# hypre-space/hypredrive

Hardware: AMD Instinct MI355X
Metric: DOF/s, AMG-PCG solve phase, 3D 7-pt Laplacian (higher is better)
Workload: dtype f64

## Files before the change

hypredrive_amd/_lib.py:

```python
import ctypes as C
import os

import numpy as np

_HERE = os.path.dirname(os.path.abspath(__file__))
_LIBPATH = os.path.join(_HERE, "lib", "libhypredrv_amd.so")
_L = None


class LibraryError(RuntimeError):
    pass


class AmgParams(C.Structure):
    _fields_ = [("coarsen_type", C.c_int), ("interp_type", C.c_int), ("pmax", C.c_int),
                ("trunc_factor", C.c_double), ("strong_th", C.c_double),
                ("max_row_sum", C.c_double), ("max_coarse_size", C.c_int),
                ("min_coarse_size", C.c_int), ("max_levels", C.c_int),
                ("relax_down", C.c_int), ("relax_up", C.c_int), ("relax_coarse", C.c_int),
                ("sweeps_down", C.c_int), ("sweeps_up", C.c_int), ("sweeps_coarse", C.c_int),
                ("relax_weight", C.c_double), ("outer_weight", C.c_double),
                ("seed", C.c_uint64), ("num_functions", C.c_int),
                ("cheby_order", C.c_int), ("cheby_eig_est", C.c_int), ("cheby_variant", C.c_int), ("cheby_scale", C.c_int),
                ("cheby_fraction", C.c_double),
# ... 43 lines not shown
                ("frelax_type", C.c_int), ("frelax_sweeps", C.c_int), ("grelax_type", C.c_int), ("grelax_sweeps", C.c_int),
                ("frelax_amg", C.POINTER(AmgParams)),
                ("ilu_tri_solve", C.c_int), ("ilu_lower_it", C.c_int), ("ilu_upper_it", C.c_int),
                ("coarse_ilu_max_iter", C.c_int), ("coarse_ilu_tri_solve", C.c_int), ("coarse_ilu_lower_it", C.c_int), ("coarse_ilu_upper_it", C.c_int),
                ("frelax_krylov", C.c_int), ("frelax_krylov_precond", C.c_int), ("frelax_kp", KrylovParams),
                ("coarse_krylov", C.c_int), ("coarse_krylov_precond", C.c_int), ("coarse_kp", KrylovParams),
                ("mgr_cycle", C.c_int), ("mgr_frelax_pos", C.c_int), ("mgr_gsmooth_pos", C.c_int), ("grelax_blocks", C.c_int),
                ("coarse_type", C.c_int), ("nonglk_max_elmts", C.c_int), ("coarse_th", C.c_double)]


SYMBOLS = [
    "hda_last_error", "hda_device_count", "hda_device_name", "hda_device_pci_bus_id", "hda_device_sync",
    "hda_amg_default_params", "hda_krylov_default_params", "hda_csr_create", "hda_csr_destroy",
    "hda_csr_dims", "hda_csr_download", "hda_lap7_create", "hda_spmv", "hda_relax", "hda_dot",
    "hda_l1_norms", "hda_strength", "hda_pmis", "hda_interp_extpi", "hda_interp_direct", "hda_rap", "hda_transpose",
    "hda_spgemm", "hda_amg_create", "hda_amg_destroy", "hda_amg_num_levels",
    "hda_last_precond_calls", "hda_amg_create_dof", "hda_format_bytes", "hda_probe_spmv", "hda_probe_read", "hda_amg_level_matrix", "hda_amg_fold_sweep", "hda_amg_level_cf", "hda_amg_complexities", "hda_amg_vcycle_bytes",
    "hda_amg_vcycle", "hda_pcg", "hda_gmres", "hda_time_kernel", "hda_solve_device",
    "hda_pcg_iteration_bytes", "hda_memory_stats", "hda_memory_cached", "hda_memory_driver_stats", "hda_memory_trim", "hda_comm_selftest", "hda_check_row_total", "hda_ilu_create", "hda_ilu_create_blocks", "hda_ilu_blocks", "hda_ilu_factors", "hda_fgmres", "hda_bicgstab", "hda_mgr_create", "hda_mgr_matrix", "hda_mgr_blk_inverses",
    "hda_probe_add", "hda_probe_read_id", "hda_borrow_hypredrv", "hda_comm_stats", "hda_comm_name", "hda_comm_size", "hda_halo_plan_host",
    "hda_amd_partitioned_levels", "hda_amd_hierarchy_levels",
    "hda_second_strength", "hda_coarsen_second_pass", "hda_interp_multipass", "hda_truncate_rows", "hda_interp_agg_two_stage",
    "hda_interp_mm_extpi", "hda_interp_extended", "hda_interp_mm_ext", "hda_interp_one_point", "hda_interp_standard", "hda_set_overlap", "hda_marker", "hda_relax_blocks", "hda_l1_norms_blocks", "hda_hmis_blocks", "hda_amg_blocks", "hda_amg_level_blocks",
    "hda_csr_form", "hda_spmv_mode", "hda_air_restriction",
    "hda_cljp", "hda_rs_blocks", "hda_falgout_blocks", "hda_measure_rnd",
    "hda_schwarz_create", "hda_schwarz_domains", "hda_schwarz_info", "hda_precond_time",
    "hda_spgemm_last_route", "hda_sort_rows_last_route",
    "hda_ams_default_amg_params", "hda_ams_create", "hda_ams_matrix", "hda_ams_info",
]


TESTRANKS_SYMBOLS = ["hda_thread_ranks_lap7", "hda_thread_world_create", "hda_thread_world_join", "hda_thread_world_leave",
                     "hda_thread_world_destroy", "hda_testranks_selftest"]
_TESTRANKS_PATH = os.path.join(os.path.dirname(_LIBPATH), "libhypredrv_amd_testranks.so")
_T = None


def load_testranks():
    global _T
    if _T is None:
        load()
        if not os.path.exists(_TESTRANKS_PATH):
            raise LibraryError(f"{_TESTRANKS_PATH} not built: run `python -c 'import __graft_entry__ as g; g.build()'`")
        _T = C.CDLL(_TESTRANKS_PATH)
    return _T


# ... 82 lines not shown
    L.hda_set_overlap.argtypes = [C.c_int]
    L.hda_set_overlap.restype = None
    L.hda_amg_num_levels.argtypes = [vp]
    L.hda_amg_level_matrix.argtypes = [vp, C.c_int, C.c_int, P(vp)]
    L.hda_amg_level_cf.argtypes = [vp, C.c_int, ip]
    L.hda_amg_fold_sweep.argtypes = [vp, C.c_int, dp, dp, dp, dp, dp]
    L.hda_amg_complexities.argtypes = [vp, dp, dp]
    L.hda_amg_vcycle_bytes.argtypes = [vp]
    L.hda_amg_vcycle_bytes.restype = C.c_double
    L.hda_amg_vcycle.argtypes = [vp, dp, dp]
    for f in (L.hda_pcg, L.hda_gmres, L.hda_fgmres, L.hda_bicgstab):
        f.argtypes = [vp, vp, P(KrylovParams), dp, dp, dp, ip, ip, dp]
    L.hda_time_kernel.argtypes = [C.c_int, vp, vp, C.c_int, dp, dp]
    L.hda_solve_device.argtypes = [vp, vp, P(KrylovParams), C.c_int, dp, C.c_int, dp, ip, dp, dp, dp, dp]
    L.hda_pcg_iteration_bytes.argtypes = [vp]
    L.hda_pcg_iteration_bytes.restype = C.c_double
    L.hda_memory_stats.argtypes = [dp, dp]
    L.hda_memory_cached.restype = C.c_double
    L.hda_memory_driver_stats.argtypes = [C.POINTER(C.c_double), C.c_int]
    L.hda_check_row_total.argtypes = [C.c_longlong, C.c_int]
    L.hda_format_bytes.argtypes = [vp, vp, dp, dp, dp, ip]
    L.hda_probe_spmv.argtypes = [vp, C.c_int]
    L.hda_csr_form.argtypes = [vp, C.c_int, ip]
    L.hda_air_restriction.argtypes = [vp, ip, C.c_int, C.c_double, C.c_double, P(vp), P(C.c_int64)]
    L.hda_spmv_mode.argtypes = [vp, C.c_int, C.c_int, C.c_double, C.c_double, dp, dp, dp, dp, dp, dp, dp, dp, dp, ip]
    L.hda_probe_read.argtypes = [dp, ip]
    L.hda_probe_add.argtypes = [vp, C.c_int, ip]
    L.hda_probe_read_id.argtypes = [C.c_int, dp, ip]
    L.hda_borrow_hypredrv.argtypes = [vp, P(vp), P(vp)]
    L.hda_comm_stats.argtypes = [dp, C.c_int]
    L.hda_comm_name.restype = C.c_char_p
    _L = L
    return L


def _check(rc):
    if rc != 0:
        raise LibraryError(f"libhypredrv_amd error {rc}: {load().hda_last_error().decode()}")


def _dp(a):
    return a.ctypes.data_as(C.POINTER(C.c_double))


def _ip(a):
    return a.ctypes.data_as(C.POINTER(C.c_int))
# ... 657 lines not shown
            "windowed": d.value in (3, 5), "value_coded": d.value in (4, 5)}


FORMS = {-1: "none", 0: "lane_group", 1: "stream", 2: "window", 3: "window_runs", 4: "coded", 5: "rowclass"}
SPMV_MODES = {"plain": 0, "plain_dot": 1, "resid": 2, "jacobi": 3, "jacobi_dot": 4, "scaled_copy": 5}


def air_restriction(A, cf, distance=2, strong_th=0.25, filter_th=0.0):
    cfa = np.ascontiguousarray(np.concatenate([np.asarray(cf, dtype=np.int32), np.zeros(1, np.int32)]), dtype=np.int32)
    st = np.zeros(5, dtype=np.int64)
    out = C.c_void_p()
    _check(load().hda_air_restriction(A.h, _ip(cfa), int(distance), float(strong_th), float(filter_th), C.byref(out),
                                      st.ctypes.data_as(C.POINTER(C.c_int64))))
    return Csr(out), dict(fallback=int(st[0]), max_m=int(st[1]), small=int(st[2]), mid=int(st[3]), large=int(st[4]))


def csr_form(A, nown=-1):
    info = np.zeros(8, dtype=np.int32)
    _check(load().hda_csr_form(A.h, nown, _ip(info)))
    return dict(kernel=FORMS[int(info[0])], lpr=int(info[1]), value_coded=bool(info[2]), escapes=int(info[3]),
                rc_esc_rows=int(info[4]), maxrow=int(info[5]), blocks=int(info[6]), vc_packed=int(info[7]))


def spmv_mode(A, mode, x, nown=-1, alpha=1.0, beta=0.0, yin=None, in_place=False, b=None, dinv=None, w=None, dinv2=None, y2=None):
    n = A.nrows
    f64 = lambda v: None if v is None else np.ascontiguousarray(v, dtype=np.float64)
    x, yin, b, dinv, w, dinv2 = f64(x), f64(yin), f64(b), f64(dinv), f64(w), f64(dinv2)
    y = yin.copy() if in_place else np.zeros(n)
    y2 = (np.zeros(n) if y2 is None else f64(y2).copy()) if dinv2 is not None else None
    p = lambda v: None if v is None else _dp(v)
    dot, taken = C.c_double(), C.c_int()
    _check(load().hda_spmv_mode(A.h, SPMV_MODES[mode], nown, alpha, beta, p(x), _dp(y) if in_place else p(yin), p(b), p(dinv), p(w),
                                p(dinv2), _dp(y), p(y2), C.byref(dot), C.byref(taken)))
    return dict(y=y, y2=y2, dot=dot.value, epilogue_taken=bool(taken.value))


def probe_spmv(A, mode):
    _check(load().hda_probe_spmv(A.h if A is not None else None, mode))


def probe_read():
    ms, n = C.c_double(), C.c_int()
    _check(load().hda_probe_read(C.byref(ms), C.byref(n)))
    return ms.value, n.value


# ... 130 lines not shown
```

hypredrive_amd/csrc/hda_capi.hip:

```cpp
#include "../../include/hypredrv_amd.h"

#include "hda_krylov.h"
#include "hda_comm.h"
#include "hda_hypre.h"

#include <chrono>
#include <cmath>
#include <cstring>

using namespace hda;

struct hda_csr_s {
   DCsr           m;
   DArray<double> rhs;
   bool           borrowed = false;
   const DCsr    *ref      = nullptr;
   const double  *rhs_ref  = nullptr;
   const HaloPlan *halo    = nullptr;
   const DCsr    &get() const { return ref ? *ref : m; }
};
struct hda_amg_s {
   Amg                                    *amg = nullptr;
   std::unique_ptr<Amg>                    owned_amg;
   std::unique_ptr<Ilu>                    ilu;
// ... 1383 lines not shown
   dx.upload(x, nc);
   dy.upload(y, nr);
   const bool in_place = yin == y;
   if (mode == HDA_SPMV_PLAIN && yin && !in_place) dyin.upload(yin, nr);
   if (b) db.upload(b, nr);
   if (dinv) ddinv.upload(dinv, nr);
   if (w) dw.upload(w, nr);
   if (mode == HDA_SPMV_SCALED_COPY)
   {
      ddinv2.upload(dinv2, nr);
      dy2.upload(y2, nr);
   }
   const double *pyin = (mode != HDA_SPMV_PLAIN || !yin) ? nullptr : in_place ? dy.data() : dyin.data();
   double        d    = 0.0;
   bool          taken = false;
   spmv_test_mode(m, mode, nown, alpha, beta, dx.data(), pyin, db.data(), ddinv.data(), dw.data(), ddinv2.data(), dy.data(), dy2.data(), &d, &taken);
   dy.download(y, nr);
   if (mode == HDA_SPMV_SCALED_COPY) dy2.download(y2, nr);
   if (dot) *dot = d;
   if (epilogue_taken) *epilogue_taken = taken;
   HDA_CATCH
}

extern "C" int hda_borrow_hypredrv(void *hypredrv, hda_csr_t *A, hda_amg_t *amg)
{
   HDA_TRY
   const DCsr     *m    = nullptr;
   const HaloPlan *halo = nullptr;
   const double   *rhs  = nullptr;
   Amg            *g    = nullptr;
   HDA_REQUIRE(hypredrv_peek(hypredrv, &m, &halo, &rhs, &g) && m, "hda_borrow_hypredrv: the object has no matrix yet");
   if (A)
   {
      auto v      = std::make_unique<hda_csr_s>();
      v->borrowed = true;
      v->ref      = m;
      v->rhs_ref  = rhs;
      v->halo     = halo;
      *A          = v.release();
   }
   if (amg)
   {
      HDA_REQUIRE(g, "hda_borrow_hypredrv: the preconditioner is not a set-up BoomerAMG hierarchy");
      auto h = std::make_unique<hda_amg_s>();
      h->amg = g;
      *amg   = h.release();
// ... 132 lines not shown
```

hypredrive_amd/csrc/hda_kernels.h:

```cpp
#pragma once

#include "hda_common.h"

namespace hda {

struct HaloPlan;


void spmv(const DCsr &A, double alpha, const double *x, double beta, const double *y_in,
          double *y_out, const HaloPlan *halo = nullptr);
bool spmv_with_scaled_copy(const DCsr &A, const double *x, double *y, const double *dinv2, double *y2, const HaloPlan *halo = nullptr);
void spmv_dot(const DCsr &A, const double *x, double *y, const double *w, int slot, const HaloPlan *halo = nullptr);
void residual(const DCsr &A, const double *x, const double *b, double *out, const HaloPlan *halo = nullptr);

void jacobi(const DCsr &A, const double *dinv, const double *b, const double *x_in,
            double *x_out, int dot_slot, const HaloPlan *halo = nullptr, const double *cdinv = nullptr);
bool class_divisors(const DCsr &A, const double *dinv, DArray<double> &table);
const unsigned char *row_classes(const DCsr &A);
void jacobi_folded(const DCsr &A, const DCsr &Pt, const double *dinv, const double *t, const double *e, const double *u, double *out);
bool spmv_foldable(const DCsr &Pt);
void jacobi_zero_guess(int n, const double *dinv, const double *b, double *x);

enum Scalar : int {
   S_GAMMA0 = 0, S_RR0 = 1, S_GAMMA1 = 2, S_RR1 = 3, S_SP = 4, S_BB = 5, S_TMP = 6, S_TMP2 = 7,
   S_GMRES = 8
};
void dot(int n, const double *x, const double *y, int slot);
void finalize(int slot, int scalar_idx);
void finalize_n(int first_slot, int nslots, int first_scalar);
void cg_update(int n, int gamma_idx, const double *p, const double *s, double *x, double *r, int rr_slot, int sp_slot = -1,
               const double *dinv0 = nullptr, double *z0 = nullptr, const unsigned char *rclass = nullptr, const double *cdinv = nullptr);
void cg_direction(int n, int gamma_old_idx, int gamma_new_idx, const double *z, double *p, int first_slot = -1, double *x = nullptr);
void cg_flush_x(int n, int gamma_idx, const double *p, double *x);
void cg_single_step(int n, int t_new, int t_old, int alpha_idx, bool first, const double *u, const double *w, double *p, double *s, double *x,
                    double *r, int rr_slot);
// ... 51 lines not shown
```

hypredrive_amd/csrc/hda_kernels.hip:

```cpp
#include "hda_kernels.h"
#include "hda_sort.h"

#include "hda_dist.h"
#include "hda_mpi_join.h"
#include <unistd.h>

#include <algorithm>
#include <cmath>
#include <cstring>
#include <limits>
#include <map>
#include <mutex>
#include <type_traits>
#include <unordered_map>
#include <rocprim/device/device_segmented_radix_sort.hpp>

namespace hda {


Context::Context()
{
   HDA_HIP(hipGetDevice(&device));
   HDA_HIP(hipStreamCreateWithFlags(&stream, hipStreamNonBlocking));
   {
// ... 987 lines not shown
            o0 = (beta == 0.0) ? alpha * sum[h] : alpha * sum[h] + beta * e0[h];
            if (DOT) acc += o0 * e1[h];
         }
         else if (MODE == MODE_RESID) o0 = e0[h] - sum[h];
         else
         {
            o0 = e2[h] + e1[h] * (e0[h] - sum[h]);
            if (DOT) acc += e0[h] * o0;
         }
         out[r] = o0;
      }
   }
   if (DOT)
   {
      acc = block_sum(acc);
      if (tid == 0)
      {
         partial[blockIdx.x] = acc;
         if (blockIdx.x + gridDim.x < kRedBlocks) partial[blockIdx.x + gridDim.x] = 0.0;
      }
   }
}

template <int MODE, bool DOT, bool SPLIT, bool CD = false>
__global__ __launch_bounds__(256) void k_spmv_rowclass(int nrows, const unsigned char *__restrict__ rclass,
                                                       const unsigned long long *__restrict__ rc_keys, const double *__restrict__ dval,
                                                       const int *__restrict__ ddelta, const int *__restrict__ rowptr,
                                                       const int *__restrict__ col, const double *__restrict__ val,
                                                       const double *__restrict__ x, double alpha, double beta, const double *yin,
                                                       const double *__restrict__ b, const double *__restrict__ dinv,
                                                       const double *__restrict__ w, double *out, double *__restrict__ partial, int nown,
                                                       const double *__restrict__ cdinv = nullptr)
{
   static_assert(!CD || MODE == MODE_JACOBI, "class divisors belong to the Jacobi sweep");
   __shared__ double sv[128 * 8];
   __shared__ int    sd[128 * 8];
   __shared__ int    sn[128];
   __shared__ double sdv[CD ? 128 : 1];
   const int tid = threadIdx.x;
   if (tid < 128)
   {
      if (CD) sdv[tid] = cdinv[tid];
      const unsigned long long key = tid < kRcSlots ? rc_keys[tid] : kRcNoKey;
      int                      n   = 0;
      for (int u = 0; u < 8; u++)
      {
         const unsigned c = (unsigned)(key >> (8 * u)) & 255u;
         const bool     on = key != kRcNoKey && c < 254u;
         sv[tid * 8 + u]   = on ? dval[c] : 0.0;
         sd[tid * 8 + u]   = on ? ddelta[c] : 0;
         n += on;
      }
      sn[tid] = n;
   }
   __syncthreads();
   const int xcd = blockIdx.x & 7, slot = blockIdx.x >> 3, nslot = gridDim.x >> 3;
   const int per = (((nrows + 7) >> 3) + 255) / 256 * 256;
   double    acc = 0.0;
   int    n_cls = 254;
   double n_e0 = 0.0, n_e1 = 0.0, n_e2 = 0.0;
   auto fetch = [&](int tile) {
      const int r = xcd * per + tile * 256 + tid;
      n_cls = 254;
      n_e0 = n_e1 = n_e2 = 0.0;
      if (tile * 256 < per && r < nrows)
      {
         n_cls = (int)rclass[r];
         if (MODE == MODE_PLAIN) { if (beta != 0.0) n_e0 = yin[r]; if (DOT) n_e1 = w[r]; }
         else if (MODE == MODE_RESID) n_e0 = b[r];
         else
         {
            n_e0 = b[r];
            n_e2 = x[r];
            if (!CD || n_cls >= 128) n_e1 = dinv[r];
         }
      }
   };
   fetch(slot);
   for (int tile = slot; tile * 256 < per; tile += nslot)
   {
      const int    r    = xcd * per + tile * 256 + tid;
      const bool   live = r < nrows;
      const int    cls  = n_cls;
      const double e0 = n_e0, e1 = (CD && cls < 128) ? sdv[cls] : n_e1, e2 = n_e2;
      double       sum = 0.0;
      fetch(tile + nslot);
      if (cls < 128)
      {
         const int     n  = sn[cls];
         const double *cv = sv + cls * 8;
         const int    *cd = sd + cls * 8;
         double        xv[8];
#pragma unroll
         for (int u = 0; u < 8; u++)
         {
            const int j = r + cd[u];
            xv[u]       = (u < n && (!SPLIT || j < nown)) ? x[j] : 0.0;
         }
#pragma unroll
         for (int u = 0; u < 8; u++)
         {
            const double t = sum + cv[u] * xv[u];
            sum            = (u < n) ? t : sum;
         }
      }
      else if (cls == 255)
      {
         for (int k = rowptr[r]; k < rowptr[r + 1]; k++)
         {
            const int j = col[k];
            if (!SPLIT || j < nown) sum += val[k] * x[j];
         }
      }
      if (live)
      {
         double o0;
         if (MODE == MODE_PLAIN)
         {
            o0 = (beta == 0.0) ? alpha * sum : alpha * sum + beta * e0;
            if (DOT) acc += o0 * e1;
         }
         else if (MODE == MODE_RESID) o0 = e0 - sum;
         else
         {
            o0 = e2 + e1 * (e0 - sum);
            if (DOT) acc += e0 * o0;
         }
         out[r] = o0;
      }
   }
   if (DOT)
   {
      acc = block_sum(acc);
      if (tid == 0)
      {
         partial[blockIdx.x] = acc;
         if (blockIdx.x + gridDim.x < kRedBlocks) partial[blockIdx.x + gridDim.x] = 0.0;
      }
   }
}
// ... 859 lines not shown
   ensure_forms(A, false);
   if (A.coded == 1) return A.rowcoded == 1 ? SpmvForm::RowClass : SpmvForm::Coded;
   const bool small = !split && A.nnz <= kSmallNnz && A.nnz > 0;
   if (A.maxrow <= kMaxRowLds && !small)
   {
      ensure_forms(A, true, split);
      if (A.win == 1) return A.win_runs ? SpmvForm::WindowRuns : SpmvForm::Window;
      return SpmvForm::Stream;
   }
   return split ? SpmvForm::None : SpmvForm::LaneGroup;
}

struct SpmvCall {
   SpmvCall(const double *x_, double *out_) : x(const_cast<double *>(x_)), out(out_) {}
   double       *x;
   double       *out;
   double        alpha = 1.0, beta = 0.0;
   const double *yin = nullptr, *b = nullptr, *dinv = nullptr, *w = nullptr;
   double       *partial = nullptr;
   const double *dinv2   = nullptr;
   double       *out2    = nullptr;
   const DCsr   *fold    = nullptr;
   const double *cdinv   = nullptr;
};

template <int MODE, bool DOT>
constexpr bool spmv_variant_ok(bool vc, bool split, bool runs, bool epi, bool fold, int pack)
{
   if (epi && (split || MODE != MODE_PLAIN || DOT)) return false;
   if (fold && (vc || runs || split || epi || MODE != MODE_JACOBI || DOT)) return false;
   if (runs && vc) return false;
   if (pack != 0 && (!vc || split || runs)) return false;
   return true;
}

template <auto... Vs>
struct OneOf {
   std::common_type_t<decltype(Vs)...> v;
};
using Flag = OneOf<false, true>;
template <class F>
static void instantiate(F &&f) { f(); }
template <class F, auto... Vs, class... Rest>
static void instantiate(F &&f, OneOf<Vs...> a, Rest... rest)
{
   const bool listed = ((a.v == Vs && (instantiate([&](auto... c) { f(std::integral_constant<decltype(Vs), Vs>{}, c...); }, rest...), true)) || ...);
// ... 2 lines not shown
[[noreturn]] static void spmv_no_kernel() { throw Error("product launch: no kernel exists for this combination of options"); }

template <int MODE, bool DOT>
static bool launch_spmv_impl(const DCsr &A_in, const SpmvCall &c, int nown = -1)
{
   const bool  split = nown >= 0;
   const bool  fold  = MODE == MODE_JACOBI && !DOT && !split && c.fold;
   const DCsr &A     = fold ? *c.fold : A_in;
   if (A.nrows == 0 && !DOT) return fold;
   const SpmvForm form = spmv_form(A, split);
   HDA_REQUIRE(form != SpmvForm::None, "split product on an operator that has no split form");
   HDA_REQUIRE(!fold || fold_form(form, A), "folded sweep armed on an operator whose storage form has no folded kernel");
   const bool stencil = form == SpmvForm::RowClass || form == SpmvForm::Coded;
   const bool runs    = form == SpmvForm::WindowRuns;
   const bool vc      = A.coded == 2 && (form == SpmvForm::Stream || form == SpmvForm::Window);
   const int pack = (vc && form == SpmvForm::Window && A.vc_pack == 1) ? (A.vc_maxesc <= kEscSlotsSmall ? kEscSlotsSmall : kEscCap) : 0;
   HDA_REQUIRE(!(split && pack), "split product on a value-coded operator with packed escapes");
   const bool     epi   = MODE == MODE_PLAIN && !DOT && !split && c.out2 && !stencil;
   const double  *dinv2 = epi ? c.dinv2 : nullptr;
   double        *out2  = epi ? c.out2 : nullptr;
   const auto    *code  = vc ? A.code.data() : nullptr;
   const double  *dict  = vc ? A.dict_val.data() : nullptr;
   const int      gmax  = split ? kOverlapGrid : kRedBlocks;
   if (stencil)
   {
      const int per  = (((A.nrows + 7) >> 3) + 255) / 256 * 256;
      const int grid = DOT ? gmax : std::min(gmax, 8 * (per / 256));
      const bool cd = MODE == MODE_JACOBI && form == SpmvForm::RowClass && c.cdinv;
      instantiate(
         [&](auto SPLIT, auto CD) {
            if constexpr (CD && MODE != MODE_JACOBI) spmv_no_kernel();
            else if (form == SpmvForm::RowClass)
               k_spmv_rowclass<MODE, DOT, SPLIT, CD><<<grid, 256, 0, STREAM>>>(A.nrows, A.rclass.data(), A.rc_keys.data(), A.dict_val.data(),
                                                                               A.dict_delta.data(), A.rowptr.data(), A.col.data(), A.val.data(), c.x,
                                                                               c.alpha, c.beta, c.yin, c.b, c.dinv, c.w, c.out, c.partial, nown,
                                                                               CD ? c.cdinv : nullptr);
            else
               k_spmv_coded_row<MODE, DOT, SPLIT><<<grid, 256, 0, STREAM>>>(A.nrows, A.rowptr.data(), A.code.data(), A.dict_val.data(),
                                                                            A.dict_delta.data(), A.col.data(), A.val.data(), c.x, c.alpha, c.beta,
                                                                            c.yin, c.b, c.dinv, c.w, c.out, c.partial, SPLIT ? nown : 0);
         },
         Flag{split}, Flag{cd});
   }
   else if (form == SpmvForm::Window || form == SpmvForm::WindowRuns)
   {
      const int     plen = kWChunk + A.maxrow;
      const size_t  wlds = sizeof(double) * (size_t)(plen + A.win_maxu);
      const int     wg   = DOT ? gmax : std::min(gmax, ((A.nwin + 7) / 8) * 8);
      const double *val  = pack ? A.vc_esc.data() : A.val.data();
      instantiate(
         [&](auto VC, auto SPLIT, auto RUNS, auto EPI, auto FOLD, auto PACK) {
            if constexpr (spmv_variant_ok<MODE, DOT>(VC, SPLIT, RUNS, EPI, FOLD, PACK))
               k_spmv_win<MODE, DOT, VC, SPLIT, RUNS, EPI, FOLD, PACK><<<wg, 256, wlds, STREAM>>>(
                  A.nwin, A.wmeta.data(), A.rowptr.data(), A.lidx.data(), A.ucol.data(), val, c.x, c.alpha, c.beta, c.yin, c.b, c.dinv, c.w, c.out,
                  c.partial, nown, plen, code, dict, kWinPf, dinv2, out2);
            else spmv_no_kernel();
         },
         Flag{vc}, Flag{split}, Flag{runs}, Flag{epi}, Flag{fold}, OneOf<0, kEscSlotsSmall, kEscCap>{pack});
   }
   else if (form == SpmvForm::Stream)
   {
      const int    grid = DOT ? gmax : std::min(gmax, ((A.nchunks + 7) / 8) * 8);
      const size_t lds  = sizeof(double) * (size_t)(kChunk + A.maxrow);
      instantiate(
         [&](auto VC, auto SPLIT, auto FOLD) {
// ... 169 lines not shown
}

void spmv(const DCsr &A, double alpha, const double *x, double beta, const double *y_in, double *y_out, const HaloPlan *halo)
{
   SpmvCall c(x, y_out);
   c.alpha = alpha;
   c.beta  = beta;
   c.yin   = y_in;
   launch_spmv<MODE_PLAIN, false>(A, halo, c);
}
bool spmv_with_scaled_copy(const DCsr &A, const double *x, double *y, const double *dinv2, double *y2, const HaloPlan *halo)
{
   SpmvCall c(x, y);
   c.dinv2 = dinv2;
   c.out2  = y2;
   return launch_spmv<MODE_PLAIN, false>(A, halo, c);
}
void spmv_dot(const DCsr &A, const double *x, double *y, const double *w, int slot, const HaloPlan *halo)
{
   SpmvCall c(x, y);
   c.w       = w;
   c.partial = Context::get().slot(slot);
   launch_spmv<MODE_PLAIN, true>(A, halo, c);
}
void residual(const DCsr &A, const double *x, const double *b, double *out, const HaloPlan *halo)
{
   SpmvCall c(x, out);
   c.b = b;
   launch_spmv<MODE_RESID, false>(A, halo, c);
}
void jacobi(const DCsr &A, const double *dinv, const double *b, const double *x_in, double *x_out, int dot_slot, const HaloPlan *halo,
            const double *cdinv)
{
   SpmvCall c(x_in, x_out);
   c.b     = b;
   c.dinv  = dinv;
   c.cdinv = cdinv;
   if (dot_slot >= 0)
   {
      c.partial = Context::get().slot(dot_slot);
      launch_spmv<MODE_JACOBI, true>(A, halo, c);
   }
   else launch_spmv<MODE_JACOBI, false>(A, halo, c);
}

__global__ __launch_bounds__(256) void k_cdinv_collect(int n, const unsigned char *__restrict__ rclass, const double *__restrict__ dinv,
// ... 213 lines not shown
               Flag{spp != nullptr}, OneOf<0, 1, 2>{zm});
}

template <bool FIN, bool XUP>
__global__ __launch_bounds__(256) void k_cg_dir(int n, double *scalars, int go, int gn, const double *__restrict__ z, double *__restrict__ p,
                                                const double *__restrict__ partials2, double *__restrict__ x)
{
   double g;
   if (FIN)
   {
      g = slot_sum_256(partials2);
      if (blockIdx.x == 0)
      {
         const double rr = slot_sum_256(partials2 + kRedBlocks);
         if (threadIdx.x == 0) { scalars[gn] = g; scalars[gn + 1] = rr; }
      }
   }
   else g = scalars[gn];
   const double beta  = g / scalars[go];
   const double alpha = XUP ? scalars[go] / scalars[S_SP] : 0.0;
   for (long i = (long)blockIdx.x * 256 + threadIdx.x; i < n; i += (long)gridDim.x * 256)
   {
      const double pi = p[i];
      if (XUP) x[i] += alpha * pi;
      p[i] = z[i] + beta * pi;
   }
}
void cg_direction(int n, int gamma_old_idx, int gamma_new_idx, const double *z, double *p, int first_slot, double *x)
{
   Context &c = Context::get();
   if (first_slot >= 0)
   {
      const int g = std::max(ew_grid(n), 1);
      if (x) k_cg_dir<true, true><<<g, 256, 0, STREAM>>>(n, c.scalars, gamma_old_idx, gamma_new_idx, z, p, c.slot(first_slot), x);
      else k_cg_dir<true, false><<<g, 256, 0, STREAM>>>(n, c.scalars, gamma_old_idx, gamma_new_idx, z, p, c.slot(first_slot), nullptr);
   }
   else if (n)
   {
      if (x) k_cg_dir<false, true><<<ew_grid(n), 256, 0, STREAM>>>(n, c.scalars, gamma_old_idx, gamma_new_idx, z, p, nullptr, x);
      else k_cg_dir<false, false><<<ew_grid(n), 256, 0, STREAM>>>(n, c.scalars, gamma_old_idx, gamma_new_idx, z, p, nullptr, nullptr);
   }
}

__global__ __launch_bounds__(256) void k_cg_flush_x(int n, const double *__restrict__ scalars, int gamma_idx, const double *__restrict__ p,
                                                    double *__restrict__ x)
{
   const double alpha = scalars[gamma_idx] / scalars[S_SP];
   for (long i = (long)blockIdx.x * 256 + threadIdx.x; i < n; i += (long)gridDim.x * 256) x[i] += alpha * p[i];
}
void cg_flush_x(int n, int gamma_idx, const double *p, double *x)
{
   if (n) k_cg_flush_x<<<ew_grid(n), 256, 0, STREAM>>>(n, Context::get().scalars, gamma_idx, p, x);
}

__global__ __launch_bounds__(256) void k_cg_single(int n, double *scalars, int t_new, int t_old, int alpha_idx, int first, const double *__restrict__ u,
                                                   const double *__restrict__ w, double *__restrict__ p, double *__restrict__ s,
                                                   double *__restrict__ x, double *__restrict__ r, double *__restrict__ partial)
{
   const double gn = scalars[t_new], delta = scalars[t_new + 2];
   double       beta = 0.0, alpha;
   if (first) alpha = gn / delta;
   else
   {
      beta  = gn / scalars[t_old];
      alpha = gn / (delta - beta * gn / scalars[alpha_idx]);
   }
   double acc = 0.0;
   for (long i = (long)blockIdx.x * 256 + threadIdx.x; i < n; i += (long)gridDim.x * 256)
   {
      const double pi = u[i] + beta * p[i], si = w[i] + beta * s[i];
      p[i]            = pi;
// ... 660 lines not shown
```

hypredrive_amd/csrc/hda_krylov.hip:

```cpp
#include "hda_krylov.h"

#include <cmath>

namespace hda {

#define g_last_precond_calls (RankState<int, 5>::get())
int last_precond_calls() { return g_last_precond_calls; }

namespace {
struct NestedScope {
   static thread_local int depth;
   DArray<double>          save;
   bool                    nested;
   static constexpr size_t kScal = Context::kNumScalars, kPart = (size_t)Context::kNumSlots * kRedBlocks;
   NestedScope() : nested(depth++ > 0)
   {
      if (!nested) return;
      Context &ctx = Context::get();
      save.alloc(kScal + kPart);
      HDA_HIP(hipMemcpyAsync(save.data(), ctx.scalars, kScal * sizeof(double), hipMemcpyDeviceToDevice, ctx.stream));
      HDA_HIP(hipMemcpyAsync(save.data() + kScal, ctx.partials, kPart * sizeof(double), hipMemcpyDeviceToDevice, ctx.stream));
   }
   ~NestedScope()
   {
      depth--;
      if (!nested) return;
      Context &ctx = Context::get();
      (void)hipMemcpyAsync(ctx.scalars, save.data(), kScal * sizeof(double), hipMemcpyDeviceToDevice, ctx.stream);
      (void)hipMemcpyAsync(ctx.partials, save.data() + kScal, kPart * sizeof(double), hipMemcpyDeviceToDevice, ctx.stream);
   }
};
thread_local int NestedScope::depth = 0;
}

double pcg_iteration_bytes(const DCsr &A, bool format)
{
   const double n = A.nrows;
   const char  *dxe = getenv("HDA_DEFER_X");
   const double vec = (format && !(dxe && atoi(dxe) == 0)) ? 24.0 * n + 40.0 * n : 48.0 * n + 24.0 * n;
   return (matrix_stream_bytes(A, format) + rowptr_stream_bytes(A, format) + 8.0 * A.ncols + 8.0 * n) + 8.0 * n + vec;
}

static KrylovResult pcg_single_reduction(const LinOp &op, const PrecondFn &M, const KrylovParams &kp, const double *b, double *x)
{
   Context     &ctx = Context::get();
   const DCsr  &A   = *op.A;
   const int    n   = A.nrows;
   KrylovResult res;
   const size_t vl = std::max<size_t>(op.veclen, 1);
   DArray<double> r(vl), u(vl), w(vl), p(vl), s(vl);
   constexpr int T0 = S_GMRES, T1 = S_GMRES + 3, S_ALPHA = S_GMRES + 6;
   auto precond = [&](const double *rr, double *zz, int slot) {
      res.precond_calls++;
      if (M) M(rr, zz, slot);
      else
      {
         copy(n, rr, zz);
         if (slot >= 0) dot(n, rr, zz, slot);
      }
   };
   dot(n, b, b, 0);
   finalize(0, S_BB);
// ... 99 lines not shown
      res.precond_calls++;
      fs.valid = false;
      if (M) M(rr, zz, slot);
      else
      {
         copy(n, rr, zz);
         if (slot >= 0) dot(n, rr, zz, slot);
      }
      HDA_REQUIRE(!fs.done, "the preconditioner ignored a first sweep it had offered to take from the caller");
      const bool mine = fs.valid && fs.n == n;
      z0_dinv = mine ? fs.dinv : nullptr;
      z0_dest = mine ? fs.dest : nullptr;
      z0_cdinv  = mine ? fs.cdinv : nullptr;
      z0_rclass = mine ? fs.rclass : nullptr;
      z0_self = mine && fs.dest == nullptr;
      fs.valid = false;
   };
   const char *ffe = getenv("HDA_FUSE_FINALIZE");
   const int   fl  = (Comm::world().size == 1) ? (ffe ? atoi(ffe) : 1) : 0;
   const bool  fin = fl >= 1, fin2 = fl >= 2;
   const char *dxe     = getenv("HDA_DEFER_X");
   const bool  defer_x = !(dxe && atoi(dxe) == 0);
   double     *xd      = defer_x ? x : nullptr;

   double bi_prod;
   if (kp.two_norm && known && !std::isnan(known->bb)) bi_prod = known->bb;
   else
   {
      if (kp.two_norm) dot(n, b, b, 0);
      else precond(b, p.data(), 0);
      finalize(0, S_BB);
      bi_prod = read_scalar(S_BB);
   }
   if (bi_prod == 0.0)
   {
      copy(n, b, x);
      ctx.sync();
      res.hist.push_back(0.0);
      return res;
   }
   double eps = kp.rtol * kp.rtol;
   {
      const double a2 = kp.atol * kp.atol / bi_prod;
      if (a2 > eps) eps = a2;
   }
   if (known && known->x_zero) copy(n, b, r.data());
   else
   {
      copy(n, x, p.data());
      residual(A, p.data(), b, r.data(), op.halo);
   }
   precond(r.data(), p.data(), 2);
   dot(n, r.data(), r.data(), 3);
   finalize_n(2, 2, S_GAMMA0);
   read_scalars_async(S_GAMMA0, 5);
   wait_event(ctx.ev);
   double i_prod = kp.two_norm ? ctx.host_scalars[S_RR0] : ctx.host_scalars[S_GAMMA0];
   res.hist.push_back(std::sqrt(std::fabs(i_prod)));
   int it = 0, x_term = -1;
   std::vector<hipEvent_t> evs;
   static const bool fuse_dots = !(getenv("HDA_FUSE_DOTS") && atoi(getenv("HDA_FUSE_DOTS")) == 0);
   while (it + 1 <= kp.max_iter)
   {
      it++;
      const int go = (it & 1) ? S_GAMMA0 : S_GAMMA1, gn = (it & 1) ? S_GAMMA1 : S_GAMMA0, rn = gn + 1;
      if (kp.profile_k1)
      {
         hipEvent_t e0, e1;
         HDA_HIP(hipEventCreate(&e0));
         HDA_HIP(hipEventCreate(&e1));
         HDA_HIP(hipEventRecord(e0, ctx.stream));
         spmv_dot(A, p.data(), s.data(), p.data(), 0, op.halo);
         HDA_HIP(hipEventRecord(e1, ctx.stream));
         evs.push_back(e0);
         evs.push_back(e1);
      }
      else
         spmv_dot(A, p.data(), s.data(), p.data(), 0, op.halo);
      if (!fin) finalize(0, S_SP);
      double *z0 = z0_dinv ? (z0_self ? s.data() : z0_dest) : nullptr;
      cg_update(n, go, p.data(), s.data(), defer_x ? nullptr : x, r.data(), 3, fin ? 0 : -1, z0_dinv, z0, z0_rclass, z0_cdinv);
      x_term = defer_x ? go : -1;
      bool stop = false;
      auto test = [&]() {
         wait_event(ctx.ev);
         const double sp = ctx.host_scalars[S_SP];
         if (sp == 0.0 || !std::isfinite(sp))
         {
            it--;
            stop = true;
            return;
         }
         i_prod = kp.two_norm ? ctx.host_scalars[rn] : ctx.host_scalars[gn];
         res.hist.push_back(std::sqrt(std::fabs(i_prod)));
         if (kp.print_level >= 2)
            printf("%5d    %e    %f    %e\n", it, res.hist.back(),
                   res.hist[res.hist.size() - 2] > 0 ? res.hist.back() / res.hist[res.hist.size() - 2] : 0.0,
                   std::sqrt(i_prod / bi_prod));
         if (i_prod / bi_prod < eps)
         {
            res.converged = true;
            stop          = true;
         }
      };
      bool near = false;
      if (kp.two_norm && res.hist.size() >= 2)
      {
         const double h1 = res.hist.back(), h0 = res.hist[res.hist.size() - 2];
         const double rho2 = (h0 > 0.0) ? (h1 / h0) * (h1 / h0) : 1.0;
         near = h1 * h1 * rho2 < 16.0 * eps * bi_prod;
      }
      if (near)
      {
         finalize(3, rn);
         read_scalars_async(S_GAMMA0, 5);
         test();
         if (stop) break;
         fs.done = z0 != nullptr;
         fs.in   = r.data();
         fs.out  = s.data();
         precond(r.data(), s.data(), 2);
         if (fin2) cg_direction(n, go, gn, s.data(), p.data(), 2, xd);
         else
         {
            finalize(2, gn);
            cg_direction(n, go, gn, s.data(), p.data(), -1, xd);
         }
         x_term = -1;
         continue;
      }
      if (!fuse_dots) finalize(3, rn);
      fs.done = z0 != nullptr;
      fs.in   = r.data();
      fs.out  = s.data();
      precond(r.data(), s.data(), 2);
      if (fin2 && fuse_dots)
      {
         cg_direction(n, go, gn, s.data(), p.data(), 2, xd);
         read_scalars_async(S_GAMMA0, 5);
      }
      else
      {
         if (fuse_dots) finalize_n(2, 2, gn);
         else finalize(2, gn);
         read_scalars_async(S_GAMMA0, 5);
         cg_direction(n, go, gn, s.data(), p.data(), -1, xd);
      }
      x_term = -1;
      test();
      if (stop) break;
   }
   fs = FirstSweepFusion();
   if (x_term >= 0) cg_flush_x(n, x_term, p.data(), x);
   ctx.sync();
   gs_free_check();
   for (size_t e = 0; e + 1 < evs.size(); e += 2)
   {
      float ms = 0.f;
      if (hipEventElapsedTime(&ms, evs[e], evs[e + 1]) == hipSuccess)
      {
         res.k1_ms_sum += ms;
         res.k1_count++;
      }
      (void)hipEventDestroy(evs[e]);
      (void)hipEventDestroy(evs[e + 1]);
   }
   res.iters     = it;
   res.final_rel = std::sqrt(std::fabs(i_prod) / bi_prod);
   if (!scope.nested) g_last_precond_calls = res.precond_calls;
   return res;
}

static KrylovResult gmres_core(bool flexible, const LinOp &op, const PrecondFn &M, const KrylovParams &kp, const double *b, double *x)
{
   NestedScope  scope;
   Context     &ctx = Context::get();
// ... 210 lines not shown
```

include/hypredrv_amd.h:

```cpp
#ifndef HYPREDRV_AMD_H
#define HYPREDRV_AMD_H

#include <stdint.h>

#ifdef __cplusplus
extern "C" {
#endif

#define HDA_OK 0
#define HDA_ERR_NO_DEVICE 1
#define HDA_ERR_RUNTIME 2
#define HDA_ERR_ARG 3

typedef struct hda_csr_s *hda_csr_t;
typedef struct hda_amg_s *hda_amg_t;

typedef struct {
   int      coarsen_type, interp_type, pmax;
   double   trunc_factor, strong_th, max_row_sum;
   int      max_coarse_size, min_coarse_size, max_levels;
   int      relax_down, relax_up, relax_coarse;
   int      sweeps_down, sweeps_up, sweeps_coarse;
   double   relax_weight, outer_weight;
   uint64_t seed;
// ... 126 lines not shown
int hda_amg_complexities(hda_amg_t h, double *grid, double *op);
double hda_amg_vcycle_bytes(hda_amg_t h);
int hda_amg_vcycle(hda_amg_t h, const double *b, double *x);

int hda_pcg(hda_csr_t A, hda_amg_t amg, const hda_krylov_params *kp, const double *b, double *x,
            double *hist, int *iters, int *converged, double *final_rel);
int hda_gmres(hda_csr_t A, hda_amg_t amg, const hda_krylov_params *kp, const double *b, double *x,
              double *hist, int *iters, int *converged, double *final_rel);
int hda_fgmres(hda_csr_t A, hda_amg_t amg, const hda_krylov_params *kp, const double *b, double *x,
              double *hist, int *iters, int *converged, double *final_rel);
int hda_bicgstab(hda_csr_t A, hda_amg_t amg, const hda_krylov_params *kp, const double *b, double *x,
              double *hist, int *iters, int *converged, double *final_rel);

int hda_time_kernel(int kind, hda_csr_t A, hda_amg_t amg, int reps, double *avg_ms, double *bytes);
int hda_last_precond_calls(void);
int hda_solve_device(hda_csr_t A, hda_amg_t amg, const hda_krylov_params *kp, int solver,
                     const double *b_host, int nsolves, double *solve_ms, int *iters,
                     double *final_rel, double *r0_norm, double *true_rel, double *k1_avg_ms);
double hda_pcg_iteration_bytes(hda_csr_t A);
int hda_format_bytes(hda_csr_t A, hda_amg_t amg, double *pcg_iteration, double *vcycle, double *spmv, int *coded);
enum { HDA_FORM_NONE = -1, HDA_FORM_LANE_GROUP = 0, HDA_FORM_STREAM = 1, HDA_FORM_WINDOW = 2, HDA_FORM_WINDOW_RUNS = 3, HDA_FORM_CODED = 4,
       HDA_FORM_ROWCLASS = 5 };
int hda_csr_form(hda_csr_t A, int nown, int *info);
enum { HDA_SPMV_PLAIN = 0, HDA_SPMV_PLAIN_DOT = 1, HDA_SPMV_RESID = 2, HDA_SPMV_JACOBI = 3, HDA_SPMV_JACOBI_DOT = 4, HDA_SPMV_SCALED_COPY = 5 };
int hda_spmv_mode(hda_csr_t A, int mode, int nown, double alpha, double beta, const double *x, const double *yin, const double *b,
                  const double *dinv, const double *w, const double *dinv2, double *y, double *y2, double *dot, int *epilogue_taken);
int hda_probe_spmv(hda_csr_t A, int mode);
int hda_probe_read(double *avg_ms, int *count);
int hda_probe_add(hda_csr_t A, int mode, int *id);
int hda_probe_read_id(int id, double *avg_ms, int *count);
int hda_borrow_hypredrv(void *hypredrv, hda_csr_t *A, hda_amg_t *amg);
int hda_halo_plan_host(int nloc, const long long *part, const long long *ghost_gids, int nghost, int *send_counts,
                       int *recv_counts, int *send_idx, int send_cap, int *send_total);
int hda_comm_stats(double out[5], int reset);
void hda_set_overlap(int mode);
const char *hda_comm_name(void);
int hda_amd_partitioned_levels(void *hypredrv);
int hda_amd_hierarchy_levels(void *hypredrv);
int         hda_comm_size(void);
int hda_comm_selftest(void);
int hda_memory_stats(double *in_use, double *peak);
double hda_memory_cached(void);
int hda_memory_driver_stats(double out[3], int reset);
int hda_memory_trim(void);
int hda_check_row_total(long long nrows, int row_len);

// ... 5 lines not shown
```

Measured before the change: 592.2 million.

## Fuse the CG direction update into the following row-class SpMV-dot kernel

The PCG loop now defers the p = z + beta*p update (and the deferred x update) and performs it inside the next SpMV-with-dot kernel for single-rank row-class operators. The new p is formed in shared memory for in-tile neighbours and recomputed from z and the old p for far neighbours, with p double-buffered. This removes one full vector pass (read z, p, x; write p, x) per iteration and one kernel launch. In exchange the SpMV reads z and p instead of p alone, adds two block barriers per tile, and needs an extra preconditioner-output buffer and p buffer. A test entry point and explicit rounding intrinsics are added so the fused and unfused paths match bitwise.

```diff
diff --git a/hypredrive_amd/_lib.py b/hypredrive_amd/_lib.py
--- a/hypredrive_amd/_lib.py
+++ b/hypredrive_amd/_lib.py
@@ -89,7 +89,7 @@
     "hda_amd_partitioned_levels", "hda_amd_hierarchy_levels",
     "hda_second_strength", "hda_coarsen_second_pass", "hda_interp_multipass", "hda_truncate_rows", "hda_interp_agg_two_stage",
     "hda_interp_mm_extpi", "hda_interp_extended", "hda_interp_mm_ext", "hda_interp_one_point", "hda_interp_standard", "hda_set_overlap", "hda_marker", "hda_relax_blocks", "hda_l1_norms_blocks", "hda_hmis_blocks", "hda_amg_blocks", "hda_amg_level_blocks",
-    "hda_csr_form", "hda_spmv_mode", "hda_air_restriction",
+    "hda_csr_form", "hda_spmv_mode", "hda_air_restriction", "hda_cg_dir_product",
     "hda_cljp", "hda_rs_blocks", "hda_falgout_blocks", "hda_measure_rnd",
     "hda_schwarz_create", "hda_schwarz_domains", "hda_schwarz_info", "hda_precond_time",
     "hda_spgemm_last_route", "hda_sort_rows_last_route",
@@ -218,6 +218,7 @@
     L.hda_format_bytes.argtypes = [vp, vp, dp, dp, dp, ip]
     L.hda_probe_spmv.argtypes = [vp, C.c_int]
     L.hda_csr_form.argtypes = [vp, C.c_int, ip]
+    L.hda_cg_dir_product.argtypes = [vp, C.c_int, dp, dp, dp, C.c_double, C.c_double, C.c_double, dp, dp, dp, ip]
     L.hda_air_restriction.argtypes = [vp, ip, C.c_int, C.c_double, C.c_double, P(vp), P(C.c_int64)]
     L.hda_spmv_mode.argtypes = [vp, C.c_int, C.c_int, C.c_double, C.c_double, dp, dp, dp, dp, dp, dp, dp, dp, dp, ip]
     L.hda_probe_read.argtypes = [dp, ip]
@@ -921,6 +922,16 @@
                 rc_esc_rows=int(info[4]), maxrow=int(info[5]), blocks=int(info[6]), vc_packed=int(info[7]))
 
 
+def cg_dir_product(A, z, p, x, gamma_old, gamma_new, sp, fused):
+    n = A.nrows
+    z, p = np.ascontiguousarray(z, dtype=np.float64), np.ascontiguousarray(p, dtype=np.float64)
+    xo = None if x is None else np.array(x, dtype=np.float64)
+    pn, s, d, can = np.zeros(n), np.zeros(n), C.c_double(), C.c_int()
+    _check(load().hda_cg_dir_product(A.h, int(bool(fused)), _dp(z), _dp(p), None if xo is None else _dp(xo), float(gamma_old), float(gamma_new),
+                                     float(sp), _dp(pn), _dp(s), C.byref(d), C.byref(can)))
+    return dict(p=pn, s=s, x=xo, dot=d.value, fusable=bool(can.value))
+
+
 def spmv_mode(A, mode, x, nown=-1, alpha=1.0, beta=0.0, yin=None, in_place=False, b=None, dinv=None, w=None, dinv2=None, y2=None):
     n = A.nrows
     f64 = lambda v: None if v is None else np.ascontiguousarray(v, dtype=np.float64)
diff --git a/hypredrive_amd/csrc/hda_capi.hip b/hypredrive_amd/csrc/hda_capi.hip
--- a/hypredrive_amd/csrc/hda_capi.hip
+++ b/hypredrive_amd/csrc/hda_capi.hip
@@ -1429,6 +1429,45 @@
    HDA_CATCH
 }
 
+extern "C" int hda_cg_dir_product(hda_csr_t A, int fused, const double *z, const double *p, double *x, double gamma_old, double gamma_new,
+                                  double sp, double *pnew, double *s, double *dot, int *fusable)
+{
+   HDA_TRY
+   HDA_REQUIRE(A && z && p && pnew && s && dot, "hda_cg_dir_product: null argument");
+   const DCsr &m = A->get();
+   HDA_REQUIRE(m.nrows == m.ncols, "hda_cg_dir_product: square operators only");
+   const bool can = spmv_dir_fusable(m, nullptr);
+   if (fusable) *fusable = can ? 1 : 0;
+   HDA_REQUIRE(!fused || can, "hda_cg_dir_product: the product of this operator has no fused direction step");
+   const size_t   n = (size_t)m.nrows;
+   Context       &ctx = Context::get();
+   DArray<double> dz, dp, dp2(n), ds(n), dx;
+   dz.upload(z, n);
+   dp.upload(p, n);
+   if (x) dx.upload(x, n);
+   const double sc[5] = {gamma_old, 0.0, gamma_new, 0.0, sp};
+   static_assert(S_GAMMA0 == 0 && S_GAMMA1 == 2 && S_SP == 4, "scalar block layout");
+   HDA_HIP(hipMemcpyAsync(ctx.scalars, sc, sizeof(sc), hipMemcpyHostToDevice, ctx.stream));
+   ctx.sync();
+   double *res = dp.data();
+   if (fused)
+   {
+      spmv_dot_dir(m, dz.data(), dp.data(), dp2.data(), ds.data(), x ? dx.data() : nullptr, S_GAMMA0, S_GAMMA1, 0);
+      res = dp2.data();
+   }
+   else
+   {
+      cg_direction((int)n, S_GAMMA0, S_GAMMA1, dz.data(), dp.data(), -1, x ? dx.data() : nullptr);
+      spmv_dot(m, dp.data(), ds.data(), dp.data(), 0, nullptr);
+   }
+   finalize(0, S_TMP);
+   *dot = read_scalar(S_TMP);
+   HDA_HIP(hipMemcpy(pnew, res, n * sizeof(double), hipMemcpyDeviceToHost));
+   ds.download(s, n);
+   if (x) dx.download(x, n);
+   HDA_CATCH
+}
+
 extern "C" int hda_borrow_hypredrv(void *hypredrv, hda_csr_t *A, hda_amg_t *amg)
 {
    HDA_TRY
diff --git a/hypredrive_amd/csrc/hda_kernels.h b/hypredrive_amd/csrc/hda_kernels.h
--- a/hypredrive_amd/csrc/hda_kernels.h
+++ b/hypredrive_amd/csrc/hda_kernels.h
@@ -11,6 +11,8 @@
           double *y_out, const HaloPlan *halo = nullptr);
 bool spmv_with_scaled_copy(const DCsr &A, const double *x, double *y, const double *dinv2, double *y2, const HaloPlan *halo = nullptr);
 void spmv_dot(const DCsr &A, const double *x, double *y, const double *w, int slot, const HaloPlan *halo = nullptr);
+bool spmv_dir_fusable(const DCsr &A, const HaloPlan *halo);
+void spmv_dot_dir(const DCsr &A, const double *z, const double *pold, double *pnew, double *y, double *x, int go, int gn, int slot);
 void residual(const DCsr &A, const double *x, const double *b, double *out, const HaloPlan *halo = nullptr);
 
 void jacobi(const DCsr &A, const double *dinv, const double *b, const double *x_in,
diff --git a/hypredrive_amd/csrc/hda_kernels.hip b/hypredrive_amd/csrc/hda_kernels.hip
--- a/hypredrive_amd/csrc/hda_kernels.hip
+++ b/hypredrive_amd/csrc/hda_kernels.hip
@@ -1033,7 +1033,13 @@
    }
 }
 
-template <int MODE, bool DOT, bool SPLIT, bool CD = false>
+struct CgDirFusion {
+   const double *z = nullptr, *pold = nullptr;
+   double       *pnew = nullptr, *x = nullptr;
+   const double *scalars = nullptr;
+   int           go = 0, gn = 0;
+};
+template <int MODE, bool DOT, bool SPLIT, bool CD = false, bool PRE = false>
 __global__ __launch_bounds__(256) void k_spmv_rowclass(int nrows, const unsigned char *__restrict__ rclass,
                                                        const unsigned long long *__restrict__ rc_keys, const double *__restrict__ dval,
                                                        const int *__restrict__ ddelta, const int *__restrict__ rowptr,
@@ -1041,9 +1047,14 @@
                                                        const double *__restrict__ x, double alpha, double beta, const double *yin,
                                                        const double *__restrict__ b, const double *__restrict__ dinv,
                                                        const double *__restrict__ w, double *out, double *__restrict__ partial, int nown,
-                                                       const double *__restrict__ cdinv = nullptr)
+                                                       const double *__restrict__ cdinv = nullptr, CgDirFusion d = CgDirFusion())
 {
    static_assert(!CD || MODE == MODE_JACOBI, "class divisors belong to the Jacobi sweep");
+   static_assert(!PRE || (MODE == MODE_PLAIN && DOT && !SPLIT), "the direction step rides on the whole plain product with its dot");
+   const double *__restrict__ dz = d.z, *__restrict__ dp = d.pold;
+   const double  dbeta  = PRE ? d.scalars[d.gn] / d.scalars[d.go] : 0.0;
+   const double  dalpha = (PRE && d.x) ? d.scalars[d.go] / d.scalars[S_SP] : 0.0;
+   __shared__ double spn[PRE ? 256 : 1];
    __shared__ double sv[128 * 8];
    __shared__ int    sd[128 * 8];
    __shared__ int    sn[128];
@@ -1077,7 +1088,13 @@
       if (tile * 256 < per && r < nrows)
       {
          n_cls = (int)rclass[r];
-         if (MODE == MODE_PLAIN) { if (beta != 0.0) n_e0 = yin[r]; if (DOT) n_e1 = w[r]; }
+         if (PRE)
+         {
+            n_e0 = dp[r];
+            n_e1 = dz[r];
+            if (d.x) n_e2 = d.x[r];
+         }
+         else if (MODE == MODE_PLAIN) { if (beta != 0.0) n_e0 = yin[r]; if (DOT) n_e1 = w[r]; }
          else if (MODE == MODE_RESID) n_e0 = b[r];
          else
          {
@@ -1095,6 +1112,13 @@
       const int    cls  = n_cls;
       const double e0 = n_e0, e1 = (CD && cls < 128) ? sdv[cls] : n_e1, e2 = n_e2;
       double       sum = 0.0;
+      const double pn = PRE ? __dadd_rn(e1, __dmul_rn(dbeta, e0)) : 0.0;
+      if (PRE)
+      {
+         __syncthreads();
+         spn[tid] = pn;
+         __syncthreads();
+      }
       fetch(tile + nslot);
       if (cls < 128)
       {
@@ -1102,11 +1126,32 @@
          const double *cv = sv + cls * 8;
          const int    *cd = sd + cls * 8;
          double        xv[8];
+         if (PRE)
+         {
+            double zv[8];
 #pragma unroll
-         for (int u = 0; u < 8; u++)
+            for (int u = 0; u < 8; u++)
+            {
+               const int  j   = r + cd[u];
+               const bool far = u < n && (unsigned)(cd[u] + tid) >= 256u;
+               zv[u]          = far ? dz[j] : 0.0;
+               xv[u]          = far ? dp[j] : 0.0;
+            }
+#pragma unroll
+            for (int u = 0; u < 8; u++)
+            {
+               const unsigned o = (unsigned)(cd[u] + tid);
+               xv[u]            = (o < 256u) ? spn[o] : __dadd_rn(zv[u], __dmul_rn(dbeta, xv[u]));
+            }
+         }
+         else
          {
-            const int j = r + cd[u];
-            xv[u]       = (u < n && (!SPLIT || j < nown)) ? x[j] : 0.0;
+#pragma unroll
+            for (int u = 0; u < 8; u++)
+            {
+               const int j = r + cd[u];
+               xv[u]       = (u < n && (!SPLIT || j < nown)) ? x[j] : 0.0;
+            }
          }
 #pragma unroll
          for (int u = 0; u < 8; u++)
@@ -1120,13 +1165,21 @@
          for (int k = rowptr[r]; k < rowptr[r + 1]; k++)
          {
             const int j = col[k];
-            if (!SPLIT || j < nown) sum += val[k] * x[j];
+            if (PRE) sum += val[k] * __dadd_rn(dz[j], __dmul_rn(dbeta, dp[j]));
+            else if (!SPLIT || j < nown) sum += val[k] * x[j];
          }
       }
       if (live)
       {
          double o0;
-         if (MODE == MODE_PLAIN)
+         if (PRE)
+         {
+            d.pnew[r] = pn;
+            if (d.x) d.x[r] = __dadd_rn(e2, __dmul_rn(dalpha, e0));
+            o0 = alpha * sum;
+            acc += o0 * pn;
+         }
+         else if (MODE == MODE_PLAIN)
          {
             o0 = (beta == 0.0) ? alpha * sum : alpha * sum + beta * e0;
             if (DOT) acc += o0 * e1;
@@ -2032,6 +2085,7 @@
    double       *out2    = nullptr;
    const DCsr   *fold    = nullptr;
    const double *cdinv   = nullptr;
+   const CgDirFusion *dir = nullptr;
 };
 
 template <int MODE, bool DOT>
@@ -2080,25 +2134,28 @@
    const auto    *code  = vc ? A.code.data() : nullptr;
    const double  *dict  = vc ? A.dict_val.data() : nullptr;
    const int      gmax  = split ? kOverlapGrid : kRedBlocks;
+   HDA_REQUIRE(!c.dir || stencil, "direction step inside a product that has no kernel for it");
    if (stencil)
    {
       const int per  = (((A.nrows + 7) >> 3) + 255) / 256 * 256;
       const int grid = DOT ? gmax : std::min(gmax, 8 * (per / 256));
       const bool cd = MODE == MODE_JACOBI && form == SpmvForm::RowClass && c.cdinv;
+      const bool pre = c.dir != nullptr;
+      HDA_REQUIRE(!pre || (form == SpmvForm::RowClass && c.beta == 0.0), "direction step inside a product that has no kernel for it");
       instantiate(
-         [&](auto SPLIT, auto CD) {
-            if constexpr (CD && MODE != MODE_JACOBI) spmv_no_kernel();
+         [&](auto SPLIT, auto CD, auto PRE) {
+            if constexpr ((CD && MODE != MODE_JACOBI) || (PRE && !(MODE == MODE_PLAIN && DOT && !SPLIT))) spmv_no_kernel();
             else if (form == SpmvForm::RowClass)
-               k_spmv_rowclass<MODE, DOT, SPLIT, CD><<<grid, 256, 0, STREAM>>>(A.nrows, A.rclass.data(), A.rc_keys.data(), A.dict_val.data(),
-                                                                               A.dict_delta.data(), A.rowptr.data(), A.col.data(), A.val.data(), c.x,
-                                                                               c.alpha, c.beta, c.yin, c.b, c.dinv, c.w, c.out, c.partial, nown,
-                                                                               CD ? c.cdinv : nullptr);
+               k_spmv_rowclass<MODE, DOT, SPLIT, CD, PRE><<<grid, 256, 0, STREAM>>>(A.nrows, A.rclass.data(), A.rc_keys.data(), A.dict_val.data(),
+                                                                                    A.dict_delta.data(), A.rowptr.data(), A.col.data(), A.val.data(),
+                                                                                    c.x, c.alpha, c.beta, c.yin, c.b, c.dinv, c.w, c.out, c.partial,
+                                                                                    nown, CD ? c.cdinv : nullptr, PRE ? *c.dir : CgDirFusion());
             else
                k_spmv_coded_row<MODE, DOT, SPLIT><<<grid, 256, 0, STREAM>>>(A.nrows, A.rowptr.data(), A.code.data(), A.dict_val.data(),
                                                                             A.dict_delta.data(), A.col.data(), A.val.data(), c.x, c.alpha, c.beta,
                                                                             c.yin, c.b, c.dinv, c.w, c.out, c.partial, SPLIT ? nown : 0);
          },
-         Flag{split}, Flag{cd});
+         Flag{split}, Flag{cd}, Flag{pre});
    }
    else if (form == SpmvForm::Window || form == SpmvForm::WindowRuns)
    {
@@ -2314,6 +2371,26 @@
    c.w       = w;
    c.partial = Context::get().slot(slot);
    launch_spmv<MODE_PLAIN, true>(A, halo, c);
+}
+bool spmv_dir_fusable(const DCsr &A, const HaloPlan *halo)
+{
+   return Comm::world().size == 1 && !halo && A.nrows > 0 && spmv_form(A, false) == SpmvForm::RowClass;
+}
+void spmv_dot_dir(const DCsr &A, const double *z, const double *pold, double *pnew, double *y, double *x, int go, int gn, int slot)
+{
+   HDA_REQUIRE(pnew != pold && pnew != z && y != z && y != pold && y != pnew, "spmv_dot_dir: pnew and y must be vectors of their own");
+   CgDirFusion d;
+   d.z       = z;
+   d.pold    = pold;
+   d.pnew    = pnew;
+   d.x       = x;
+   d.scalars = Context::get().scalars;
+   d.go      = go;
+   d.gn      = gn;
+   SpmvCall c(pold, y);
+   c.partial = Context::get().slot(slot);
+   c.dir     = &d;
+   launch_spmv<MODE_PLAIN, true>(A, nullptr, c);
 }
 void residual(const DCsr &A, const double *x, const double *b, double *out, const HaloPlan *halo)
 {
@@ -2573,8 +2650,8 @@
    for (long i = (long)blockIdx.x * 256 + threadIdx.x; i < n; i += (long)gridDim.x * 256)
    {
       const double pi = p[i];
-      if (XUP) x[i] += alpha * pi;
-      p[i] = z[i] + beta * pi;
+      if (XUP) x[i] = __dadd_rn(x[i], __dmul_rn(alpha, pi));
+      p[i] = __dadd_rn(z[i], __dmul_rn(beta, pi));
    }
 }
 void cg_direction(int n, int gamma_old_idx, int gamma_new_idx, const double *z, double *p, int first_slot, double *x)
@@ -2597,7 +2674,7 @@
                                                     double *__restrict__ x)
 {
    const double alpha = scalars[gamma_idx] / scalars[S_SP];
-   for (long i = (long)blockIdx.x * 256 + threadIdx.x; i < n; i += (long)gridDim.x * 256) x[i] += alpha * p[i];
+   for (long i = (long)blockIdx.x * 256 + threadIdx.x; i < n; i += (long)gridDim.x * 256) x[i] = __dadd_rn(x[i], __dmul_rn(alpha, p[i]));
 }
 void cg_flush_x(int n, int gamma_idx, const double *p, double *x)
 {
diff --git a/hypredrive_amd/csrc/hda_krylov.hip b/hypredrive_amd/csrc/hda_krylov.hip
--- a/hypredrive_amd/csrc/hda_krylov.hip
+++ b/hypredrive_amd/csrc/hda_krylov.hip
@@ -37,7 +37,14 @@
 {
    const double n = A.nrows;
    const char  *dxe = getenv("HDA_DEFER_X");
-   const double vec = (format && !(dxe && atoi(dxe) == 0)) ? 24.0 * n + 40.0 * n : 48.0 * n + 24.0 * n;
+   const bool   dx  = !(dxe && atoi(dxe) == 0);
+   if (format && n > 0)
+   {
+      const char *fde = getenv("HDA_FUSE_DIR"), *ffe = getenv("HDA_FUSE_FINALIZE");
+      if (!(fde && atoi(fde) == 0) && !(ffe && atoi(ffe) >= 2) && spmv_dir_fusable(A, nullptr))
+         return matrix_stream_bytes(A, true) + rowptr_stream_bytes(A, true) + (dx ? 48.0 * n + 24.0 * n : 32.0 * n + 48.0 * n);
+   }
+   const double vec = (format && dx) ? 24.0 * n + 40.0 * n : 48.0 * n + 24.0 * n;
    return (matrix_stream_bytes(A, format) + rowptr_stream_bytes(A, format) + 8.0 * A.ncols + 8.0 * n) + 8.0 * n + vec;
 }
 
@@ -183,6 +190,17 @@
    const char *dxe     = getenv("HDA_DEFER_X");
    const bool  defer_x = !(dxe && atoi(dxe) == 0);
    double     *xd      = defer_x ? x : nullptr;
+   const char *fde      = getenv("HDA_FUSE_DIR");
+   const bool  fuse_dir = !(fde && atoi(fde) == 0) && !fin2 && n > 0 && spmv_dir_fusable(A, op.halo);
+   DArray<double> p2, zb;
+   if (fuse_dir)
+   {
+      p2.alloc(vl);
+      zb.alloc(vl);
+   }
+   double *pc = p.data(), *pn = p2.data();
+   double *zv = fuse_dir ? zb.data() : s.data();
+   int     dir_go = -1, dir_gn = -1;
 
    double bi_prod;
    if (kp.two_norm && known && !std::isnan(known->bb)) bi_prod = known->bb;
@@ -221,6 +239,26 @@
    int it = 0, x_term = -1;
    std::vector<hipEvent_t> evs;
    static const bool fuse_dots = !(getenv("HDA_FUSE_DOTS") && atoi(getenv("HDA_FUSE_DOTS")) == 0);
+   auto product = [&]() {
+      if (dir_go >= 0)
+      {
+         spmv_dot_dir(A, zv, pc, pn, s.data(), xd, dir_go, dir_gn, 0);
+         std::swap(pc, pn);
+         dir_go = -1;
+         x_term = -1;
+      }
+      else spmv_dot(A, pc, s.data(), pc, 0, op.halo);
+   };
+   auto direction = [&](int go, int gn, int first_slot) {
+      if (fuse_dir)
+      {
+         dir_go = go;
+         dir_gn = gn;
+         return;
+      }
+      cg_direction(n, go, gn, zv, pc, first_slot, xd);
+      x_term = -1;
+   };
    while (it + 1 <= kp.max_iter)
    {
       it++;
@@ -231,16 +269,16 @@
          HDA_HIP(hipEventCreate(&e0));
          HDA_HIP(hipEventCreate(&e1));
          HDA_HIP(hipEventRecord(e0, ctx.stream));
-         spmv_dot(A, p.data(), s.data(), p.data(), 0, op.halo);
+         product();
          HDA_HIP(hipEventRecord(e1, ctx.stream));
          evs.push_back(e0);
          evs.push_back(e1);
       }
       else
-         spmv_dot(A, p.data(), s.data(), p.data(), 0, op.halo);
+         product();
       if (!fin) finalize(0, S_SP);
-      double *z0 = z0_dinv ? (z0_self ? s.data() : z0_dest) : nullptr;
-      cg_update(n, go, p.data(), s.data(), defer_x ? nullptr : x, r.data(), 3, fin ? 0 : -1, z0_dinv, z0, z0_rclass, z0_cdinv);
+      double *z0 = z0_dinv ? (z0_self ? zv : z0_dest) : nullptr;
+      cg_update(n, go, pc, s.data(), defer_x ? nullptr : x, r.data(), 3, fin ? 0 : -1, z0_dinv, z0, z0_rclass, z0_cdinv);
       x_term = defer_x ? go : -1;
       bool stop = false;
       auto test = [&]() {
@@ -279,25 +317,24 @@
          if (stop) break;
          fs.done = z0 != nullptr;
          fs.in   = r.data();
-         fs.out  = s.data();
-         precond(r.data(), s.data(), 2);
-         if (fin2) cg_direction(n, go, gn, s.data(), p.data(), 2, xd);
+         fs.out  = zv;
+         precond(r.data(), zv, 2);
+         if (fin2) direction(go, gn, 2);
          else
          {
             finalize(2, gn);
-            cg_direction(n, go, gn, s.data(), p.data(), -1, xd);
+            direction(go, gn, -1);
          }
-         x_term = -1;
          continue;
       }
       if (!fuse_dots) finalize(3, rn);
       fs.done = z0 != nullptr;
       fs.in   = r.data();
-      fs.out  = s.data();
-      precond(r.data(), s.data(), 2);
+      fs.out  = zv;
+      precond(r.data(), zv, 2);
       if (fin2 && fuse_dots)
       {
-         cg_direction(n, go, gn, s.data(), p.data(), 2, xd);
+         direction(go, gn, 2);
          read_scalars_async(S_GAMMA0, 5);
       }
       else
@@ -305,14 +342,13 @@
          if (fuse_dots) finalize_n(2, 2, gn);
          else finalize(2, gn);
          read_scalars_async(S_GAMMA0, 5);
-         cg_direction(n, go, gn, s.data(), p.data(), -1, xd);
-      }
-      x_term = -1;
+         direction(go, gn, -1);
+      }
       test();
       if (stop) break;
    }
    fs = FirstSweepFusion();
-   if (x_term >= 0) cg_flush_x(n, x_term, p.data(), x);
+   if (x_term >= 0) cg_flush_x(n, x_term, pc, x);
    ctx.sync();
    gs_free_check();
    for (size_t e = 0; e + 1 < evs.size(); e += 2)
diff --git a/include/hypredrv_amd.h b/include/hypredrv_amd.h
--- a/include/hypredrv_amd.h
+++ b/include/hypredrv_amd.h
@@ -172,6 +172,8 @@
 enum { HDA_FORM_NONE = -1, HDA_FORM_LANE_GROUP = 0, HDA_FORM_STREAM = 1, HDA_FORM_WINDOW = 2, HDA_FORM_WINDOW_RUNS = 3, HDA_FORM_CODED = 4,
        HDA_FORM_ROWCLASS = 5 };
 int hda_csr_form(hda_csr_t A, int nown, int *info);
+int hda_cg_dir_product(hda_csr_t A, int fused, const double *z, const double *p, double *x, double gamma_old, double gamma_new, double sp,
+                       double *pnew, double *s, double *dot, int *fusable);
 enum { HDA_SPMV_PLAIN = 0, HDA_SPMV_PLAIN_DOT = 1, HDA_SPMV_RESID = 2, HDA_SPMV_JACOBI = 3, HDA_SPMV_JACOBI_DOT = 4, HDA_SPMV_SCALED_COPY = 5 };
 int hda_spmv_mode(hda_csr_t A, int mode, int nown, double alpha, double beta, const double *x, const double *yin, const double *b,
                   const double *dinv, const double *w, const double *dinv2, double *y, double *y2, double *dot, int *epilogue_taken);
```

Measured after the change: 596.5 million (median of 6 runs). No clear change (+0.7%).
